# AkshayJha22/Cross-Sectional-Momentum-Strategy-Replication-Backtesting-Framework

Measured on AMD Instinct MI355X. Metric: asset-periods backtested/sec (1/2/4/8 GPU) + % HBM peak BW; decile match %, higher is better.
Workload: dtype f64

## Files before the change

### cross-sectional-momentum-strategy-replication-backtesting-framework_amd/csrc/scan.h

```cpp
#pragma once
#include "csm_common.h"

struct ScanLane {
  double pff;
  double psff;
  int head;
  int prev;
};

__device__ __forceinline__ void scan_init(ScanLane& s, double* ring, int RS, int W,
                                          const double* __restrict__ carry, int64_t N,
                                          int64_t a, bool live) {
  if (live && carry) {
    for (int k = 0; k < W; ++k) ring[k * RS] = carry[(int64_t)k * N + a];
    s.pff = carry[(int64_t)W * N + a];
    s.psff = carry[(int64_t)(W + 1) * N + a];
  } else {
    for (int k = 0; k < W; ++k) ring[k * RS] = qnan();
    s.pff = qnan();
    s.psff = qnan();
  }
  s.head = 0;
  s.prev = -1;
}

__device__ __forceinline__ double ffill(double x, double last) { return isnan_d(x) ? last : x; }

__device__ __forceinline__ double price_step(double x, double& pff) {
  const double nx = ffill(x, pff);
  const double ret = nx / pff - 1.0;
  pff = nx;
  return ret;
}

__device__ __forceinline__ void lds_push(double* ring, int RS, int W, int& head, double fct) {
  ring[head * RS] = fct;
  head = (head + 1 == W) ? 0 : head + 1;
}

template <int JC = 0>
__device__ __forceinline__ double lds_prod(const double* ring, int RS, int W, int J, int idx) {
  double acc = ring[idx * RS];
  if constexpr (JC > 0) {
    double f[JC];
#pragma unroll
    for (int k = 1; k < JC; ++k) {
      idx = (idx + 1 == W) ? 0 : idx + 1;
      f[k] = ring[idx * RS];
    }
#pragma unroll
    for (int k = 1; k < JC; ++k) acc = acc * f[k];
  } else {
    for (int k = 1; k < J; ++k) {
      idx = (idx + 1 == W) ? 0 : idx + 1;
      acc = acc * ring[idx * RS];
    }
  }
  return acc;
}

template <int RW>
__device__ __forceinline__ void reg_push(double (&f)[RW], double fct, bool on = true) {
#pragma unroll
  for (int k = 0; k + 1 < RW; ++k) f[k] = on ? f[k + 1] : f[k];
  f[RW - 1] = on ? fct : f[RW - 1];
}

template <int RW>
__device__ __forceinline__ double reg_prod(const double (&f)[RW], int J) {
  double acc = f[0];
#pragma unroll
  for (int k = 1; k < RW; ++k)
    if (k < J) acc = acc * f[k];
  return acc;
}

template <int RW, bool FIX>
__device__ __forceinline__ double mj_window(const double (&f)[RW], int q, int lo, int hi) {
  if constexpr (FIX) {
    constexpr int Jq[4] = {3, 6, 9, 12};
    double acc = 0.0;
#pragma unroll
    for (int qq = 0; qq < 4; ++qq) {
      if (qq != q) continue;
      const int l = RW - Jq[qq] - 1;
      double a = f[l];
#pragma unroll
      for (int k = l + 1; k < RW - 1; ++k) a = a * f[k];
      acc = a;
    }
    return acc;
  }
  double acc = 1.0;
#pragma unroll
  for (int k = 0; k < RW; ++k) acc = (k >= lo && k < hi) ? acc * f[k] : acc;
  return acc;
}

__device__ __forceinline__ double subset_ret(double ps_new, double psff) {
  return ps_new / psff - 1.0;
}

template <class Settle>
__device__ __forceinline__ bool rank_step(double x, double mom, int m, double& psff, int& prev,
                                          Settle settle) {
  const bool ranked = !isnan_d(mom);
  const double ps_new = ffill(x, psff);
  if (prev >= 0) settle(prev, subset_ret(ps_new, psff));
  if (ranked) {
    psff = ps_new;
    prev = m;
    return false;
  }
  prev = -1;
  return true;
}

__device__ __forceinline__ double pending_finish(double x, double psff) {
  return is_absent(x) ? qnan() : subset_ret(ffill(x, psff), psff);
}

__device__ __forceinline__ void scan_finish(ScanLane& s, double* ring, int RS, int W, int64_t N,
                                            int64_t a, double* __restrict__ NR,
                                            const double* __restrict__ next_pm,
                                            double* __restrict__ carry_out) {
  if (s.prev >= 0)
    NR[(int64_t)s.prev * N + a] = next_pm ? pending_finish(next_pm[a], s.psff) : qnan();
  if (carry_out) {
    int idx = s.head;
    for (int k = 0; k < W; ++k) {
      carry_out[(int64_t)k * N + a] = ring[idx * RS];
      idx = (idx + 1 == W) ? 0 : idx + 1;
    }
    carry_out[(int64_t)W * N + a] = s.pff;
    carry_out[(int64_t)(W + 1) * N + a] = s.psff;
  }
}

template <int JC = 0>
__device__ __forceinline__ double lds_push_mom(ScanLane& s, double* ring, int RS, int W, int J,
                                               double fct) {
  lds_push(ring, RS, W, s.head, fct);
  return lds_prod<JC>(ring, RS, W, J, s.head) - 1.0;
}

template <class Ring>
__device__ __forceinline__ double scan_step_on(ScanLane& s, double x, int m, int64_t N, int64_t a,
                                               double* __restrict__ R, double* __restrict__ M,
                                               double* __restrict__ NR, Ring push_prod) {
  const double NaN = qnan();
  const int64_t o = (int64_t)m * N + a;
  if (is_absent(x)) {
    if (R) R[o] = NaN;
    M[o] = NaN;
    NR[o] = NaN;
    return NaN;
  }
  const double ret = price_step(x, s.pff);
  const double mom = push_prod(1.0 + ret);
  if (rank_step(x, mom, m, s.psff, s.prev,
                [&](int row, double nr) { NR[(int64_t)row * N + a] = nr; }))
    NR[o] = NaN;
  if (R) R[o] = ret;
  M[o] = mom;
  return mom;
}

__device__ __forceinline__ void store_pair(double* p, double v0, double v1) {
  *reinterpret_cast<double2*>(p) = make_double2(v0, v1);
}

__device__ __forceinline__ void store_next_ret_pair(double* __restrict__ NR, int64_t N,
                                                    int64_t a0, int64_t o, const int (&wp)[2],
                                                    const double (&vp)[2], const bool (&wc)[2]) {
  const double NaN = qnan();
  if (wp[0] >= 0 && wp[0] == wp[1]) {
    store_pair(NR + (int64_t)wp[0] * N + a0, vp[0], vp[1]);
  } else {
    if (wp[0] >= 0) NR[(int64_t)wp[0] * N + a0] = vp[0];
    if (wp[1] >= 0) NR[(int64_t)wp[1] * N + a0 + 1] = vp[1];
  }
  if (wc[0] && wc[1]) {
    store_pair(NR + o, NaN, NaN);
  } else {
    if (wc[0]) NR[o] = NaN;
    if (wc[1]) NR[o + 1] = NaN;
  }
}

__device__ __forceinline__ void chunk_range(int T_m, int G, int g, int& m0, int& m1) {
  const int base = T_m / G, rem = T_m % G;
  m0 = g * base + (g < rem ? g : rem);
  m1 = m0 + base + (g < rem ? 1 : 0);
}

template <int JC = 0>
__device__ __forceinline__ double scan_step(ScanLane& s, double x, int m, double* ring, int RS,
                                            int W, int J, int64_t N, int64_t a,
                                            double* __restrict__ R, double* __restrict__ M,
                                            double* __restrict__ NR) {
  return scan_step_on(s, x, m, N, a, R, M, NR,
                      [&](double fct) { return lds_push_mom<JC>(s, ring, RS, W, J, fct); });
}

template <int JC = 0>
__device__ __forceinline__ void scan_step_pair(ScanLane (&s)[2], const double (&x)[2], int m,
                                               double* ring0, int RS, int W, int J, int64_t N,
                                               int64_t a0, double* __restrict__ R,
                                               double* __restrict__ M, double* __restrict__ NR,
                                               double (&mom)[2]) {
  const double NaN = qnan();
  double ret[2];
  int wp[2];
  double vp[2];
  bool wc[2];
#pragma unroll
  for (int c = 0; c < 2; ++c) {
    wp[c] = -1;
    vp[c] = NaN;
    if (is_absent(x[c])) {
      ret[c] = NaN; mom[c] = NaN; wc[c] = true;
      continue;
    }
    ret[c] = price_step(x[c], s[c].pff);
    mom[c] = lds_push_mom<JC>(s[c], ring0 + c, RS, W, J, 1.0 + ret[c]);
    const bool ranked = !isnan_d(mom[c]);
    const double ps_new = ffill(x[c], s[c].psff);
    if (s[c].prev >= 0) { wp[c] = s[c].prev; vp[c] = subset_ret(ps_new, s[c].psff); }
    if (ranked) {
      s[c].psff = ps_new;
      s[c].prev = m;
      wc[c] = false;
    } else {
      s[c].prev = -1;
      wc[c] = true;
    }
  }
  const int64_t o = (int64_t)m * N + a0;
  if (R) store_pair(R + o, ret[0], ret[1]);
  store_pair(M + o, mom[0], mom[1]);
  store_next_ret_pair(NR, N, a0, o, wp, vp, wc);
}

__device__ __forceinline__ void scan_shadow(ScanLane& s, double x, int m, double* ring, int RS,
                                            int W, int J) {
  if (is_absent(x)) return;
  const double ret = price_step(x, s.pff);
  const double mom = lds_push_mom(s, ring, RS, W, J, 1.0 + ret);
  rank_step(x, mom, m, s.psff, s.prev, [](int, double) {});
}

template <int VEC> struct RowT;
template <> struct RowT<1> { typedef double T; };
template <> struct RowT<2> { typedef double2 T; };
__device__ __forceinline__ double comp(double v, int) { return v; }
__device__ __forceinline__ double comp(double2 v, int k) { return k == 0 ? v.x : v.y; }

template <int WR, int JC = 0>
__device__ __forceinline__ double scan_step_reg(ScanLane& s, double x, int m, double (&fr)[WR],
                                                int J, int64_t N, int64_t a,
                                                double* __restrict__ R, double* __restrict__ M,
                                                double* __restrict__ NR) {
  return scan_step_on(s, x, m, N, a, R, M, NR, [&](double fct) {
    reg_push(fr, fct);
    return reg_prod(fr, JC > 0 ? JC : J) - 1.0;
  });
}
```

### cross-sectional-momentum-strategy-replication-backtesting-framework_amd/csrc/signal.hip

```cpp
#include "csm_common.h"
#include "scan.h"
#include "shard.h"


#define PROBE_M 8
#define PROBE_DEN 8
__device__ __forceinline__ bool tail_probe(const double* __restrict__ P,
                                           const int64_t* __restrict__ month_start, int T_m,
                                           int64_t N, int64_t T_d) {
  static_assert(PROBE_M == 8, "the month spacing is a shift");
  const int lane = threadIdx.x & 63;
  const int64_t cs = N / 128;
  double x[PROBE_M][2];
  bool in[PROBE_M];
#pragma unroll
  for (int i = 0; i < PROBE_M; ++i) {
    const int m = (int)(((int64_t)(2 * i + 1) * T_m) >> 4);
    const int64_t d0 = month_start[m] < 0 ? 0 : month_start[m];
    const int64_t d1 = month_start[m + 1] < T_d ? month_start[m + 1] : T_d;
    in[i] = d1 > d0;
#pragma unroll
    for (int j = 0; j < 2; ++j)
      x[i][j] = in[i] ? P[(d1 - 1) * N + (2 * lane + j) * cs] : 0.0;
  }
  int gaps = 0, tot = 0;
#pragma unroll
  for (int i = 0; i < PROBE_M; ++i)
#pragma unroll
    for (int j = 0; j < 2; ++j) {
      gaps += __popcll(__ballot(in[i] && !(x[i][j] == x[i][j])));
      tot += in[i] ? 64 : 0;
    }
  return gaps * PROBE_DEN <= tot;
}

struct HaloArgs {
  int H, F, before, after;
  uint8_t* flags;
};
#define HALO_BATCH 8
template <int MAXD, int VEC, int NBUF, int BW, bool SH, bool BL, int JC = 0, bool HALO = false>
__global__ __launch_bounds__(64 * BW) void k_signal(
    const double* __restrict__ P, const int64_t* __restrict__ month_start, int T_m, int64_t N,
    int J, int skip, double* __restrict__ PMo, double* __restrict__ R, double* __restrict__ M,
    double* __restrict__ NR, const double* __restrict__ carry, const double* __restrict__ next_pm,
    double* __restrict__ carry_out, int64_t T_d, uint16_t* __restrict__ IDS, HaloArgs ha,
    int probe) {
  static_assert(!HALO || (SH && VEC == 2), "the halo prologue: shard passes, paired lanes");
  if (probe && tail_probe(P, month_start, T_m, N, T_d)) return;
  typedef typename RowT<VEC>::T VT;
  extern __shared__ __attribute__((aligned(16))) double ring_lds[];
  const int W = J + skip;
  const int tid = threadIdx.x;
  const int64_t a0 = ((int64_t)blockIdx.x * 64 * BW + tid) * VEC;
  const bool live = a0 < N;
  const int RS = 64 * VEC * BW;
  ScanLane sl[VEC];
  int* shc = reinterpret_cast<int*>(ring_lds + W * RS);
#pragma unroll
  for (int k = 0; k < VEC; ++k) {
    scan_init(sl[k], ring_lds + VEC * tid + k, RS, W, HALO ? nullptr : carry, N, a0 + k, live);
    if (SH) {
      shc[VEC * tid + k] = 0;
      shc[RS + VEC * tid + k] = -1;
      shc[2 * RS + VEC * tid + k] = -1;
    }
  }
  double npmh[VEC];
  if constexpr (HALO) {
    constexpr int HU = HALO_BATCH;
    const int64_t* ms = month_start;
    const int H = ha.H, F = ha.F, HF = H + F;
    const int64_t as = live ? a0 : 0;
    const int lane = tid & 63, wv = tid >> 6;
    const int64_t aw = a0 - 2 * lane;
    double* hpw = ring_lds + (size_t)W * RS + (size_t)(3 * RS) / 2;
    uint16_t* wl = reinterpret_cast<uint16_t*>(hpw + HU * RS) + wv * (HU * 128);
    int nh[VEC], fv[VEC], lv[VEC];
#pragma unroll
    for (int c = 0; c < VEC; ++c) { nh[c] = 0; fv[c] = -1; lv[c] = -1; npmh[c] = absent_val(); }
    for (int j0 = 0; j0 < HF; j0 += HU) {
      double2 xl[HU];
#pragma unroll
      for (int u = 0; u < HU; ++u) {
        const int j = j0 + u;
        const int m = j < H ? j : j + T_m;
        xl[u] = make_double2(absent_val(), absent_val());
        if (j < HF) {
          const int64_t d0 = ms[m], d1 = ms[m + 1];
          if (d1 > d0) xl[u] = *reinterpret_cast<const double2*>(P + (d1 - 1) * N + as);
        }
      }
      int nit = 0;
#pragma unroll
      for (int u = 0; u < HU; ++u) {
        *reinterpret_cast<double2*>(hpw + u * RS + 2 * tid) = xl[u];
#pragma unroll
        for (int c = 0; c < VEC; ++c) {
          const double x = comp(xl[u], c);
          const bool need = live && j0 + u < HF && !(x == x);
          const uint64_t mk = __ballot(need);
          if (need) wl[nit + lane_prefix(mk)] = (uint16_t)(u * 128 + 2 * lane + c);
          nit += __popcll(mk);
        }
      }
      __builtin_amdgcn_wave_barrier();
      for (int it0 = 0; it0 < nit; it0 += 128) {
        int item[2], u[2];
        int64_t d0[2], d1[2];
        double xs[2][HALO_WALK];
#pragma unroll
        for (int h = 0; h < 2; ++h) {
          const int it = it0 + 64 * h + lane;
          item[h] = it < nit ? (int)wl[it] : -1;
          u[h] = item[h] >> 7;
          const int j = j0 + (item[h] < 0 ? 0 : u[h]);
          const int m = j < H ? j : j + T_m;
          d0[h] = ms[m];
          d1[h] = ms[m + 1];
          const int64_t a = aw + (item[h] & 127);
#pragma unroll
          for (int k = 0; k < HALO_WALK; ++k) {
            const int64_t d = d1[h] - 2 - k;
            xs[h][k] = (item[h] >= 0 && d >= d0[h]) ? P[d * N + a] : absent_val();
          }
        }
#pragma unroll
        for (int h = 0; h < 2; ++h) {
          if (item[h] < 0) continue;
          const int64_t a = aw + (item[h] & 127);
          const double xlast = hpw[u[h] * RS + 128 * wv + (item[h] & 127)];
          bool p = !is_absent(xlast), got = false;
          double x = 0.0;
#pragma unroll
          for (int k = 0; k < HALO_WALK; ++k) {
            if (!got && xs[h][k] == xs[h][k]) { x = xs[h][k]; got = true; }
            p |= !is_absent(xs[h][k]);
          }
          if (!got && d1[h] - 1 - HALO_WALK > d0[h]) {
            const double y = halo_month_price(P, d0[h], d1[h] - 1 - HALO_WALK, N, a);
            if (y == y) { x = y; got = true; }
            p |= !is_absent(y);
          }
          hpw[u[h] * RS + 128 * wv + (item[h] & 127)] = got ? x : (p ? qnan() : absent_val());
        }
      }
      __syncthreads();
#pragma unroll
      for (int u = 0; u < HU; ++u) {
        const int j = j0 + u;
        if (j >= HF) break;
#pragma unroll
        for (int c = 0; c < VEC; ++c) {
          const double x = hpw[u * RS + 2 * tid + c];
          if (j < H) {
            if (live && !is_absent(x)) {
              if (!isnan_d(x)) { if (fv[c] < 0) fv[c] = nh[c]; lv[c] = nh[c]; }
              ++nh[c];
              scan_shadow(sl[c], x, j, ring_lds + VEC * tid + c, RS, W, J);
            }
          } else if (is_absent(npmh[c])) {
            npmh[c] = x;
          }
        }
      }
      __syncthreads();
    }
#pragma unroll
    for (int c = 0; c < VEC; ++c) {
      sl[c].prev = -1;
      uint8_t fl = 0;
      if (ha.before && !(fv[c] >= 0 && lv[c] - fv[c] >= W)) fl |= 1;
      if (ha.after && is_absent(npmh[c])) fl |= 2;
      if (live && ha.flags) ha.flags[a0 + c] = fl;
    }
    month_start += H;
  }
  const double* base = P + (live ? a0 : 0);
  const int64_t rstride = N;
  static_assert(!BL || VEC == 2, "buffer loads: paired lanes");
  const int voff = (int)((live ? a0 : 0) * 8);
  auto load_month = [&](VT (&buf)[MAXD], int mm) {
    mm = mm < T_m ? mm : T_m - 1;
    const int64_t f0 = month_start[mm], nn = month_start[mm + 1] - f0;
    if constexpr (BL) {
      typedef unsigned int u32x4 __attribute__((ext_vector_type(4)));
      const __amdgpu_buffer_rsrc_t rs = __builtin_amdgcn_make_buffer_rsrc(
          (void*)(P + f0 * N), (short)0, (int)(nn * N * 8), 0x00020000);
#pragma unroll
      for (int k = 0; k < MAXD; ++k) {
        const u32x4 w = __builtin_amdgcn_raw_buffer_load_b128(rs, voff + k * (int)(N * 8), 0, 0);
        buf[k] = *reinterpret_cast<const VT*>(&w);
      }
    } else {
      const int64_t pad = nn > 0 ? nn - 1 : (f0 > 0 ? -1 : 0);
#pragma unroll
      for (int k = 0; k < MAXD; ++k)
        buf[k] = *reinterpret_cast<const VT*>(base + (f0 + (k < nn ? k : pad)) * rstride);
    }
  };
  auto process = [&](const VT (&X)[MAXD], int m) {
    double pm[VEC];
    const int nnm = (int)(month_start[m + 1] - month_start[m]);
#pragma unroll
    for (int c = 0; c < VEC; ++c) {
      double last = 0.0;
      bool p = false, v = false;
#pragma unroll
      for (int k = 0; k < MAXD; ++k) {
        const double x = comp(X[k], c);
        const bool in = BL ? k < nnm : nnm > 0;
        const bool ok = in && x == x;
        p |= in && !is_absent(x);
        v |= ok;
        last = ok ? x : last;
      }
      pm[c] = p ? (v ? last : qnan()) : absent_val();
      if (SH && p) {
        int* q = shc + VEC * tid + c;
        q[0] += 1;
        if (q[RS] < 0) q[RS] = m;
        q[2 * RS] = m;
      }
    }
    if (live) {
      if (PMo && (!SH || shard_pm_kept(m, T_m, W))) {
        if (VEC == 2) *reinterpret_cast<double2*>(PMo + (int64_t)m * N + a0) = make_double2(pm[0], pm[VEC - 1]);
        else PMo[(int64_t)m * N + a0] = pm[0];
      }
      double mom[VEC];
      if constexpr (VEC == 2) {
        scan_step_pair<JC>(reinterpret_cast<ScanLane (&)[2]>(sl), reinterpret_cast<const double (&)[2]>(pm),
                       m, ring_lds + VEC * tid, RS, W, J, N, a0, R, M, NR,
                       reinterpret_cast<double (&)[2]>(mom));
      } else {
#pragma unroll
        for (int c = 0; c < VEC; ++c)
          mom[c] = scan_step(sl[c], pm[c], m, ring_lds + VEC * tid + c, RS, W, J, N, a0 + c, R, M, NR);
      }
      if (IDS) {
        if (VEC == 2)
          *reinterpret_cast<uint32_t*>(IDS + (int64_t)m * N + a0) =
              csm_fid(mom[0]) | (csm_fid(mom[VEC - 1]) << 16);
        else
          IDS[(int64_t)m * N + a0] = (uint16_t)csm_fid(mom[0]);
      }
    }
  };
  static_assert(NBUF == 2 || NBUF == 4, "two or four month buffers");
  VT A[MAXD], B[MAXD];
  if (NBUF == 2) {
    load_month(A, 0);
    for (int m = 0; m < T_m; m += 2) {
      load_month(B, m + 1);
      process(A, m);
      load_month(A, m + 2);
      if (m + 1 < T_m) process(B, m + 1);
    }
  } else {
    VT C[MAXD], D[MAXD];
    load_month(A, 0);
    load_month(B, 1);
    load_month(C, 2);
    for (int m = 0; m < T_m; m += 4) {
      load_month(D, m + 3);
      process(A, m);
      load_month(A, m + 4);
      if (m + 1 < T_m) process(B, m + 1);
      load_month(B, m + 5);
      if (m + 2 < T_m) process(C, m + 2);
      load_month(C, m + 6);
      if (m + 3 < T_m) process(D, m + 3);
    }
  }
  if (live) {
#pragma unroll
    for (int k = 0; k < VEC; ++k) {
      if constexpr (HALO) {
        if (sl[k].prev >= 0)
          NR[(int64_t)sl[k].prev * N + a0 + k] = pending_finish(npmh[k], sl[k].psff);
      } else {
        scan_finish(sl[k], ring_lds + VEC * tid + k, RS, W, N, a0 + k, NR, next_pm,
                    SH ? nullptr : carry_out);
      }
      if (SH) {
        const int* q = shc + VEC * tid + k;
        carry_out[a0 + k] = (double)q[0];
        carry_out[N + a0 + k] = (double)sl[k].prev;
        carry_out[2 * N + a0 + k] = sl[k].psff;
        carry_out[3 * N + a0 + k] = (double)q[RS];
        carry_out[4 * N + a0 + k] = (double)q[2 * RS];
      }
    }
  }
}

#define TAIL_U 8
#define TAIL_BACK 3

template <int MAXD, int BW, int JC>
__global__ __launch_bounds__(64 * BW) void k_signal_tail(
    const double* __restrict__ P, const int64_t* __restrict__ month_start, int T_m, int64_t N,
    int J, int skip, double* __restrict__ PMo, double* __restrict__ R, double* __restrict__ M,
    double* __restrict__ NR, const double* __restrict__ carry, const double* __restrict__ next_pm,
    double* __restrict__ carry_out, int64_t T_d, uint16_t* __restrict__ IDS,
    int probe) {
  if (probe && !tail_probe(P, month_start, T_m, N, T_d)) return;
  extern __shared__ __attribute__((aligned(16))) double ring_lds[];
  constexpr int U = TAIL_U, RS = 64 * BW, WA = 64;
  const int W = J + skip;
  const int tid = threadIdx.x, lane = tid & 63, wv = tid >> 6;
  const int64_t a0 = (int64_t)blockIdx.x * RS + tid;
  const bool live = a0 < N;
  const int64_t as = live ? a0 : 0;
  const int64_t aw = a0 - lane;
  const int64_t* ms = month_start;
  double* hp = ring_lds + (size_t)W * RS;
  double* hpw = hp + WA * wv;
  uint16_t* wl = reinterpret_cast<uint16_t*>(hp + U * RS) + wv * (2 * U * WA);
  uint16_t* wl2 = wl + U * WA;
  ScanLane sl;
  scan_init(sl, ring_lds + tid, RS, W, carry, N, a0, live);
  if (aw >= N) return;

  auto month_rows = [&](int m, int64_t& d0, int64_t& d1) {
    d0 = ms[m];
    d1 = ms[m + 1];
    d0 = d0 < 0 ? 0 : d0;
    d1 = d1 < T_d ? d1 : T_d;
  };
  auto load_last = [&](double (&xl)[U], int m0) {
#pragma unroll
    for (int u = 0; u < U; ++u) {
      xl[u] = absent_val();
      if (m0 + u < T_m) {
        int64_t d0, d1;
        month_rows(m0 + u, d0, d1);
        if (d1 > d0) xl[u] = P[(d1 - 1) * N + as];
      }
    }
  };
  auto fold = [&](double y, double& x, bool& got, bool& p) {
    if (!got && y == y) { x = y; got = true; }
    p |= !is_absent(y);
  };
  constexpr int K = MAXD - 1;
  struct Walk {
    int item, u, col;
    int64_t d0, d1;
    bool act;
  };
  auto issue = [&](auto& xs, Walk& w, const uint16_t* list, int it, int n, int m0) {
    constexpr int KK = sizeof(xs) / sizeof(double);
    w.act = it < n;
    w.item = w.act ? (int)list[it] : 0;
    w.u = w.item / WA;
    w.col = w.item % WA;
    month_rows(m0 + w.u, w.d0, w.d1);
    const int64_t a = aw + w.col;
#pragma unroll
    for (int k = 0; k < KK; ++k) {
      const int64_t d = w.d1 - 2 - k;
      xs[k] = (w.act && d >= w.d0) ? P[d * N + a] : absent_val();
    }
  };
  auto finish_back = [&](const double (&xs)[TAIL_BACK], const Walk& w, int& nb) {
    bool p = true, got = false;
    double x = 0.0;
#pragma unroll
    for (int k = 0; k < TAIL_BACK; ++k) fold(xs[k], x, got, p);
    const bool more = w.act && !got && w.d1 - 2 - TAIL_BACK >= w.d0;
    if (w.act && !more) hpw[w.u * RS + w.col] = got ? x : qnan();
    const uint64_t mk = __ballot(more);
    if (more) wl2[nb + lane_prefix(mk)] = (uint16_t)w.item;
    nb += __popcll(mk);
  };
  auto finish_month = [&](const double (&xs)[K], const Walk& w) {
    bool p = !is_absent(hpw[w.u * RS + w.col]), got = false;
    double x = 0.0;
#pragma unroll
    for (int k = 0; k < K; ++k) fold(xs[k], x, got, p);
    if (w.act) hpw[w.u * RS + w.col] = got ? x : (p ? qnan() : absent_val());
  };
  auto walk_months = [&](int i0, int n, int m0) {
    double XS[K], XT[K];
    Walk wb, wc;
    const bool two = i0 + 64 < n;
    issue(XS, wb, wl2, i0 + lane, n, m0);
    if (two) issue(XT, wc, wl2, i0 + 64 + lane, n, m0);
    finish_month(XS, wb);
    if (two) finish_month(XT, wc);
  };

  double xa[U], xb[U];
  load_last(xa, 0);
  for (int m0 = 0; m0 < T_m; m0 += U) {
    load_last(xb, m0 + U);
    int na = 0, nb = 0;
#pragma unroll
    for (int u = 0; u < U; ++u) {
      hp[u * RS + tid] = xa[u];
      bool in = false;
      if (m0 + u < T_m) {
        int64_t d0, d1;
        month_rows(m0 + u, d0, d1);
        in = d1 > d0;
      }
      const double x = xa[u];
      const bool need = live && in && !(x == x);
      const bool nb_ = need && is_absent(x), na_ = need && !nb_;
      const uint64_t mka = __ballot(na_), mkb = __ballot(nb_);
      const int item = u * WA + lane;
      if (na_) wl[na + lane_prefix(mka)] = (uint16_t)item;
      if (nb_) wl2[nb + lane_prefix(mkb)] = (uint16_t)item;
      na += __popcll(mka);
      nb += __popcll(mkb);
    }
    __builtin_amdgcn_wave_barrier();
    if (na + nb > 0) {
      double xs[TAIL_BACK];
      Walk wa;
      int db = nb < 128 ? nb : 128;
      issue(xs, wa, wl, lane, na, m0);
      walk_months(0, db, m0);
      finish_back(xs, wa, nb);
      for (int it0 = 64; it0 < na; it0 += 64) {
        issue(xs, wa, wl, it0 + lane, na, m0);
        finish_back(xs, wa, nb);
      }
      __builtin_amdgcn_wave_barrier();
      for (; db < nb; db += 128) walk_months(db, nb, m0);
    }
    __builtin_amdgcn_wave_barrier();
#pragma unroll 1
    for (int u = 0; u < U; ++u) {
      const int m = m0 + u;
      if (m >= T_m) break;
      if (!live) continue;
      const double pm = hp[u * RS + tid];
      if (PMo) PMo[(int64_t)m * N + a0] = pm;
      const double mom = scan_step<JC>(sl, pm, m, ring_lds + tid, RS, W, J, N, a0, R, M, NR);
      if (IDS) IDS[(int64_t)m * N + a0] = (uint16_t)csm_fid(mom);
    }
    __builtin_amdgcn_wave_barrier();
#pragma unroll
    for (int u = 0; u < U; ++u) xa[u] = xb[u];
  }
  if (live) scan_finish(sl, ring_lds + tid, RS, W, N, a0, NR, next_pm, carry_out);
}

static int g_tune_signal_vec = 2;
static int g_tune_signal_bwf = 0;
static int g_tune_signal_tail = 2;
static int g_tune_signal_j12 = 1;
#define SIGNAL_BWF_MIN_N (180 * 512)
static const TuneKnob g_knobs[] = {
    {"signal_vec", &g_tune_signal_vec, [](int v) { return v == 1 || v == 2; }},
    {"signal_bwf", &g_tune_signal_bwf, [](int v) { return v == 0 || v == 1 || v == 4; }},
    {"signal_j12", &g_tune_signal_j12, [](int v) { return v == 0 || v == 1; }},
    {"signal_tail", &g_tune_signal_tail, [](int v) { return v >= 0 && v <= 2; }},
};
int csm_tune_signal(const char* key, int value) { return tune_set(g_knobs, key, value); }

int signal_launch(csm_ctx* ctx, const char* who, const double* P, int64_t T_d, int64_t N,
                  const int64_t* month_start, int32_t T_m, int32_t max_month_days, int32_t J,
                  int32_t skip, double* PM, double* R, double* M, double* NR, const double* carry,
                  const double* next_pm, double* carry_out, bool sh, uint16_t* ids,
                  const HaloArgs* halo) {
  int r = prep(ctx);
  if (r) return r;
  if (sh && (!PM || !carry_out || T_m < 1))
    return set_err(ctx, CSM_E_INVAL, "%s: a shard pass needs PM and state, and at least one month",
                   who);
  if (!P || !month_start || !M || !NR || N <= 0 || T_d < 0 || T_m < 0 || J < 1 || skip < 0 ||
      J + skip > 256 || max_month_days < 1)
    return set_err(ctx, CSM_E_INVAL, "%s: bad arguments (N=%lld T_m=%d J=%d skip=%d)", who,
                   (long long)N, T_m, J, skip);
  if (max_month_days > 32)
    return set_err(ctx, CSM_E_INVAL, "%s: months longer than 32 days are not supported "
                   "(use csm_month_end + csm_momentum)", who);
  if (T_m == 0) return CSM_OK;
  if (T_d == 0)
    return set_err(ctx, CSM_E_INVAL, "%s: %d months and no day row", who, T_m);
  const int W = J + skip;
  const bool can2 = (N % 2 == 0) && aligned16(P) && (!PM || aligned16(PM)) && aligned16(M) &&
                    aligned16(NR) && (!R || aligned16(R));
  const int vec = (g_tune_signal_vec == 1 || !can2) ? 1 : 2;
  const size_t tlds = (size_t)(W + TAIL_U) * 128 * sizeof(double) + (size_t)2 * TAIL_U * 128 * sizeof(uint16_t);
  int tail = (!sh && !halo && can2 && tlds <= 160 * 1024) ? g_tune_signal_tail : 0;
  if (tail == 2 && N < (int64_t)SIGNAL_BWF_MIN_N) tail = 1;
  int probe_ = tail == 2;
  if (tail != 0) {
    const bool d23 = max_month_days <= 23, j12 = J == 12;
    const void* fn =
        d23 ? (j12 ? (const void*)k_signal_tail<23, 2, 12> : (const void*)k_signal_tail<23, 2, 0>)
            : (j12 ? (const void*)k_signal_tail<32, 2, 12> : (const void*)k_signal_tail<32, 2, 0>);
    if (tlds > 65536)
      HIP_CHECK(ctx, hipFuncSetAttribute(fn, hipFuncAttributeMaxDynamicSharedMemorySize, (int)tlds));
    const unsigned blocks = (unsigned)((N + 127) / 128);
    int T_m_ = T_m, J_ = J, skip_ = skip;
    int64_t N_ = N, T_d_ = T_d;
    void* args[] = {(void*)&P, (void*)&month_start, &T_m_, &N_, &J_, &skip_, (void*)&PM, (void*)&R,
                    (void*)&M, (void*)&NR, (void*)&carry, (void*)&next_pm, (void*)&carry_out, &T_d_,
                    (void*)&ids, &probe_};
    HIP_CHECK(ctx, hipLaunchKernel(fn, dim3(blocks), dim3(128), args, tlds, ctx->stream));
    LAUNCH_CHECK(ctx, who);
    if (tail == 1) return CSM_OK;
  }
  const bool fits4 = vec == 2 && max_month_days <= 23 && N * 8 * 32 < ((int64_t)1 << 31);
  const bool wide4 = fits4 && (g_tune_signal_bwf == 4 ||
                               (g_tune_signal_bwf == 0 && N >= (int64_t)SIGNAL_BWF_MIN_N));
  const int bw = wide4 ? 4 : 1;
  const size_t lds = (size_t)W * 64 * vec * bw * sizeof(double) +
                     (sh ? (size_t)3 * 64 * vec * bw * sizeof(int) : 0) +
                     (halo ? (size_t)HALO_BATCH * 64 * vec * bw * sizeof(double) +
                             (size_t)bw * HALO_BATCH * 128 * sizeof(uint16_t) : 0);
  const unsigned blocks = (unsigned)((N / vec + 64 * bw - 1) / (64 * bw));
  const void* fn = nullptr;
#define SIG1(V, SH_)                                                                            \
  (max_month_days <= 23 && V == 2 ? (const void*)k_signal<23, V, 4, 1, SH_, false>              \
   : max_month_days <= 24         ? (const void*)k_signal<24, V, 4, 1, SH_, false>              \
                                  : (const void*)k_signal<32, V, 4, 1, SH_, false>)
  const bool j12 = sh && J == 12 && g_tune_signal_j12;
  if (halo && !(sh && wide4))
    return set_err(ctx, CSM_E_INVAL, "%s: the fused halo prologue runs in the wide shard kernel "
                   "(even N >= %d, months of <= 23 days); use csm_shard_halo + "
                   "csm_signal_shard_halo", who, SIGNAL_BWF_MIN_N);
  if (halo)
    fn = j12 ? (const void*)k_signal<23, 2, 2, 4, true, true, 12, true>
             : (const void*)k_signal<23, 2, 2, 4, true, true, 0, true>;
  else if (wide4 && j12)
    fn = (const void*)k_signal<23, 2, 2, 4, true, true, 12>;
  else if (wide4)
    fn = sh ? (const void*)k_signal<23, 2, 2, 4, true, true> : (const void*)k_signal<23, 2, 2, 4, false, true>;
  else if (vec == 2)
    fn = sh ? SIG1(2, true) : SIG1(2, false);
  else
    fn = sh ? SIG1(1, true) : SIG1(1, false);
#undef SIG1
  if (lds > 65536)
    HIP_CHECK(ctx, hipFuncSetAttribute(fn, hipFuncAttributeMaxDynamicSharedMemorySize, (int)lds));
  {
    int T_m_ = T_m, J_ = J, skip_ = skip;
    int64_t N_ = N, T_d_ = T_d;
    HaloArgs ha = halo ? *halo : HaloArgs{0, 0, 0, 0, nullptr};
    void* args[] = {(void*)&P, (void*)&month_start, &T_m_, &N_, &J_, &skip_, (void*)&PM, (void*)&R,
                    (void*)&M, (void*)&NR, (void*)&carry, (void*)&next_pm, (void*)&carry_out, &T_d_,
                    (void*)&ids, (void*)&ha, &probe_};
    HIP_CHECK(ctx, hipLaunchKernel(fn, dim3(blocks), dim3(64 * bw), args, lds, ctx->stream));
  }
  LAUNCH_CHECK(ctx, who);
  return CSM_OK;
}

extern "C" {

int csm_signal(csm_ctx* ctx, const double* P, int64_t T_d, int64_t N, const int64_t* month_start,
               int32_t T_m, int32_t max_month_days, int32_t J, int32_t skip, double* PM, double* R,
               double* M, double* NR, const double* carry, const double* next_pm,
               double* carry_out) {
  return signal_launch(ctx, "csm_signal", P, T_d, N, month_start, T_m, max_month_days, J,
                       skip, PM, R, M, NR, carry, next_pm, carry_out);
}

int csm_signal_ids(csm_ctx* ctx, const double* P, int64_t T_d, int64_t N,
                   const int64_t* month_start, int32_t T_m, int32_t max_month_days,
                   int32_t min_month_days, int32_t J, int32_t skip, double* PM, double* R,
                   double* M, double* NR, uint16_t* ids) {
  if (!ids || (N % 4) != 0 || ((uintptr_t)ids & 7u) != 0)
    return set_err(ctx, CSM_E_INVAL, "csm_signal_ids: ids must be non-NULL and 8-B aligned, N %% 4 == 0 "
                   "(N=%lld)", (long long)N);
  (void)min_month_days;
  return signal_launch(ctx, "csm_signal_ids", P, T_d, N, month_start, T_m, max_month_days, J,
                       skip, PM, R, M, NR, nullptr, nullptr, nullptr, false, ids);
}

int csm_signal_shard(csm_ctx* ctx, const double* P, int64_t T_d, int64_t N,
                     const int64_t* month_start, int32_t T_m, int32_t max_month_days, int32_t J,
                     int32_t skip, double* PM, double* R, double* M, double* NR, double* state) {
  return signal_launch(ctx, "csm_signal_shard", P, T_d, N, month_start, T_m,
                       max_month_days, J, skip, PM, R, M, NR, nullptr, nullptr, state, true);
}

int csm_signal_shard_ids(csm_ctx* ctx, const double* P, int64_t T_d, int64_t N,
                         const int64_t* month_start, int32_t T_m, int32_t max_month_days,
                         int32_t J, int32_t skip, double* PM, double* R, double* M, double* NR,
                         double* state, uint16_t* ids) {
  if (!ids || (N % 4) != 0 || ((uintptr_t)ids & 7u) != 0)
    return set_err(ctx, CSM_E_INVAL, "csm_signal_shard_ids: needs ids, N %% 4 == 0, 8-B aligned ids");
  return signal_launch(ctx, "csm_signal_shard_ids", P, T_d, N, month_start, T_m,
                       max_month_days, J, skip, PM, R, M, NR, nullptr, nullptr, state, true, ids);
}

int csm_signal_halo(csm_ctx* ctx, const double* P, int64_t T_d, int64_t N,
                    const int64_t* month_start, int32_t H, int32_t T_m, int32_t F, int32_t before,
                    int32_t after, int32_t max_month_days, int32_t J, int32_t skip, double* PM,
                    double* R, double* M, double* NR, double* state, uint16_t* ids,
                    uint8_t* flags) {
  if (!flags || H < 0 || F < 0 || F > 8 || J + skip > 64)
    return set_err(ctx, CSM_E_INVAL, "csm_signal_halo: bad arguments (flags [N], H >= 0, "
                   "0 <= F <= 8, J + skip <= 64)");
  if (ids && ((N % 4) != 0 || ((uintptr_t)ids & 7u) != 0))
    return set_err(ctx, CSM_E_INVAL, "csm_signal_halo: ids need N %% 4 == 0, 8-B alignment");
  const HaloArgs ha{H, F, before ? 1 : 0, after ? 1 : 0, flags};
  return signal_launch(ctx, "csm_signal_halo", P, T_d, N, month_start, T_m, max_month_days, J,
                       skip, PM, R, M, NR, nullptr, nullptr, state, true, ids, &ha);
}

int csm_signal_shard_halo(csm_ctx* ctx, const double* P, int64_t T_d, int64_t N,
                          const int64_t* month_start, int32_t T_m, int32_t max_month_days,
                          int32_t J, int32_t skip, const double* carry, const double* next_pm,
                          double* PM, double* R, double* M, double* NR, double* state,
                          uint16_t* ids) {
  if (!carry || !next_pm)
    return set_err(ctx, CSM_E_INVAL, "csm_signal_shard_halo: needs the halo's carry and next_pm");
  if (ids && ((N % 4) != 0 || ((uintptr_t)ids & 7u) != 0))
    return set_err(ctx, CSM_E_INVAL, "csm_signal_shard_halo: ids need N %% 4 == 0, 8-B alignment");
  return signal_launch(ctx, "csm_signal_shard_halo", P, T_d, N, month_start, T_m, max_month_days,
                       J, skip, PM, R, M, NR, carry, next_pm, state, true, ids);
}

}
```

Measured before the change: 822.5 billion.

## Batch the tail kernel's per-month scan across eight months with an enlarged ring

Replaces the serial per-month scan_step loop in the tail kernel with scan_step_batch, which processes U=8 months at once. It precomputes head/tail ring indices, pushes all factors, then computes the J-window products for all months in parallel. The LDS ring is enlarged to S=W+U-1 slots so that the batched pushes do not overwrite windows still being read, and the ring is moved after the month/list buffers. The last-price loads are also made branchless so the U gathers can issue together. The goal is to break the month-to-month dependency chain and expose ILP, at the cost of more LDS, more registers and more complex wraparound logic.

```diff
diff --git a/cross-sectional-momentum-strategy-replication-backtesting-framework_amd/csrc/scan.h b/cross-sectional-momentum-strategy-replication-backtesting-framework_amd/csrc/scan.h
--- a/cross-sectional-momentum-strategy-replication-backtesting-framework_amd/csrc/scan.h
+++ b/cross-sectional-momentum-strategy-replication-backtesting-framework_amd/csrc/scan.h
@@ -26,9 +26,10 @@
 
 __device__ __forceinline__ double ffill(double x, double last) { return isnan_d(x) ? last : x; }
 
+__device__ __forceinline__ double price_ret(double nx, double pff) { return nx / pff - 1.0; }
 __device__ __forceinline__ double price_step(double x, double& pff) {
   const double nx = ffill(x, pff);
-  const double ret = nx / pff - 1.0;
+  const double ret = price_ret(nx, pff);
   pff = nx;
   return ret;
 }
@@ -123,14 +124,15 @@
 __device__ __forceinline__ void scan_finish(ScanLane& s, double* ring, int RS, int W, int64_t N,
                                             int64_t a, double* __restrict__ NR,
                                             const double* __restrict__ next_pm,
-                                            double* __restrict__ carry_out) {
+                                            double* __restrict__ carry_out, int S = 0) {
+  if (S == 0) S = W;
   if (s.prev >= 0)
     NR[(int64_t)s.prev * N + a] = next_pm ? pending_finish(next_pm[a], s.psff) : qnan();
   if (carry_out) {
     int idx = s.head;
     for (int k = 0; k < W; ++k) {
       carry_out[(int64_t)k * N + a] = ring[idx * RS];
-      idx = (idx + 1 == W) ? 0 : idx + 1;
+      idx = (idx + 1 == S) ? 0 : idx + 1;
     }
     carry_out[(int64_t)W * N + a] = s.pff;
     carry_out[(int64_t)(W + 1) * N + a] = s.psff;
@@ -201,6 +203,137 @@
                                             double* __restrict__ NR) {
   return scan_step_on(s, x, m, N, a, R, M, NR,
                       [&](double fct) { return lds_push_mom<JC>(s, ring, RS, W, J, fct); });
+}
+
+template <int U>
+__device__ __forceinline__ void held(double (&v)[U]) {
+#pragma unroll
+  for (int u = 0; u < U; ++u) asm volatile("" : "+v"(v[u]));
+}
+
+template <int U, int JC = 0>
+__device__ __forceinline__ void scan_step_batch(ScanLane& s, const double (&x)[U], int m0, int nm,
+                                                bool live, double* ring, int RS, int W, int S,
+                                                int J, int64_t N, int64_t a,
+                                                double* __restrict__ R, double* __restrict__ M,
+                                                double* __restrict__ NR, double (&mom)[U]) {
+  const double NaN = qnan();
+  const int SB = S * RS;
+  bool pr[U];
+  double nx[U], den[U];
+  int tl[U], hd[U];
+  {
+    double pff = s.pff;
+    int head = s.head * RS;
+    int tail = head + W * RS;
+    tail = tail >= SB ? tail - SB : tail;
+#pragma unroll
+    for (int u = 0; u < U; ++u) {
+      pr[u] = live && u < nm && !is_absent(x[u]);
+      nx[u] = ffill(x[u], pff);
+      den[u] = pff;
+      pff = pr[u] ? nx[u] : pff;
+      tl[u] = tail;
+      const int h1 = head + RS == SB ? 0 : head + RS, t1 = tail + RS == SB ? 0 : tail + RS;
+      head = pr[u] ? h1 : head;
+      tail = pr[u] ? t1 : tail;
+      hd[u] = head;
+    }
+    s.pff = pff;
+    s.head = head / RS;
+  }
+  double ret[U];
+#pragma unroll
+  for (int u = 0; u < U; ++u) ret[u] = price_ret(nx[u], den[u]);
+  held(ret);
+#pragma unroll
+  for (int u = 0; u < U; ++u) ring[tl[u]] = 1.0 + ret[u];
+  double acc[U];
+  if constexpr (JC > 0) {
+    const double* p0[U];
+    const double* p1[U];
+    int kw[U];
+#pragma unroll
+    for (int u = 0; u < U; ++u) {
+      p0[u] = ring + hd[u];
+      p1[u] = p0[u] - SB;
+      kw[u] = SB - hd[u];
+      acc[u] = *p0[u];
+    }
+    double f[U], g[U];
+#pragma unroll
+    for (int u = 0; u < U; ++u) f[u] = (RS >= kw[u] ? p1[u] : p0[u])[RS];
+#pragma unroll
+    for (int k = 1; k < JC; ++k) {
+#pragma unroll
+      for (int u = 0; u < U; ++u)
+        g[u] = k + 1 < JC ? ((k + 1) * RS >= kw[u] ? p1[u] : p0[u])[(k + 1) * RS] : 0.0;
+#pragma unroll
+      for (int u = 0; u < U; ++u) acc[u] = acc[u] * f[u];
+      held(acc);
+#pragma unroll
+      for (int u = 0; u < U; ++u) f[u] = g[u];
+    }
+  } else {
+    int ix[U];
+#pragma unroll
+    for (int u = 0; u < U; ++u) {
+      ix[u] = hd[u];
+      acc[u] = ring[ix[u]];
+    }
+    for (int k = 1; k < J; ++k) {
+#pragma unroll
+      for (int u = 0; u < U; ++u) {
+        ix[u] = ix[u] + RS == SB ? 0 : ix[u] + RS;
+        acc[u] = acc[u] * ring[ix[u]];
+      }
+      held(acc);
+    }
+  }
+#pragma unroll
+  for (int u = 0; u < U; ++u) mom[u] = pr[u] ? acc[u] - 1.0 : NaN;
+  int srow[U];
+  double snum[U], sden[U];
+  bool unr[U];
+  {
+    double psff = s.psff;
+    int prev = s.prev;
+#pragma unroll
+    for (int u = 0; u < U; ++u) {
+      const bool ranked = pr[u] && !isnan_d(mom[u]);
+      snum[u] = ffill(x[u], psff);
+      sden[u] = psff;
+      srow[u] = pr[u] ? prev : -1;
+      unr[u] = !ranked;
+      psff = ranked ? snum[u] : psff;
+      prev = pr[u] ? (ranked ? m0 + u : -1) : prev;
+    }
+    s.psff = psff;
+    s.prev = prev;
+  }
+  double nr[U];
+  bool other = false;
+#pragma unroll
+  for (int u = 0; u < U; ++u)
+    other |= srow[u] >= 0 && !(__double_as_longlong(snum[u]) == __double_as_longlong(nx[u]) &&
+                               __double_as_longlong(sden[u]) == __double_as_longlong(den[u]));
+  if (__ballot(other) != 0) {
+#pragma unroll
+    for (int u = 0; u < U; ++u) nr[u] = subset_ret(snum[u], sden[u]);
+    held(nr);
+  } else {
+#pragma unroll
+    for (int u = 0; u < U; ++u) nr[u] = ret[u];
+  }
+#pragma unroll
+  for (int u = 0; u < U; ++u) {
+    if (!(live && u < nm)) continue;
+    const int64_t o = (int64_t)(m0 + u) * N + a;
+    if (R) R[o] = pr[u] ? ret[u] : NaN;
+    M[o] = mom[u];
+    if (srow[u] >= 0) NR[(int64_t)srow[u] * N + a] = nr[u];
+    if (unr[u]) NR[o] = NaN;
+  }
 }
 
 template <int JC = 0>
diff --git a/cross-sectional-momentum-strategy-replication-backtesting-framework_amd/csrc/signal.hip b/cross-sectional-momentum-strategy-replication-backtesting-framework_amd/csrc/signal.hip
--- a/cross-sectional-momentum-strategy-replication-backtesting-framework_amd/csrc/signal.hip
+++ b/cross-sectional-momentum-strategy-replication-backtesting-framework_amd/csrc/signal.hip
@@ -306,19 +306,22 @@
     double* __restrict__ carry_out, int64_t T_d, uint16_t* __restrict__ IDS,
     int probe) {
   if (probe && !tail_probe(P, month_start, T_m, N, T_d)) return;
-  extern __shared__ __attribute__((aligned(16))) double ring_lds[];
+  extern __shared__ __attribute__((aligned(16))) double tail_lds[];
   constexpr int U = TAIL_U, RS = 64 * BW, WA = 64;
-  const int W = J + skip;
+  const int W = J + skip, S = W + U - 1;
   const int tid = threadIdx.x, lane = tid & 63, wv = tid >> 6;
   const int64_t a0 = (int64_t)blockIdx.x * RS + tid;
   const bool live = a0 < N;
   const int64_t as = live ? a0 : 0;
   const int64_t aw = a0 - lane;
   const int64_t* ms = month_start;
-  double* hp = ring_lds + (size_t)W * RS;
+  double* hp = tail_lds;
   double* hpw = hp + WA * wv;
   uint16_t* wl = reinterpret_cast<uint16_t*>(hp + U * RS) + wv * (2 * U * WA);
   uint16_t* wl2 = wl + U * WA;
+  constexpr int LISTS = 2 * U * RS * (int)sizeof(uint16_t) / (int)sizeof(double);
+  static_assert(U * RS + LISTS >= (JC - 1) * RS, "a wrapped window's pointer leaves the array");
+  double* ring_lds = hp + U * RS + LISTS;
   ScanLane sl;
   scan_init(sl, ring_lds + tid, RS, W, carry, N, a0, live);
   if (aw >= N) return;
@@ -330,15 +333,18 @@
     d1 = d1 < T_d ? d1 : T_d;
   };
   auto load_last = [&](double (&xl)[U], int m0) {
+    int64_t d1[U];
+    bool in[U];
 #pragma unroll
     for (int u = 0; u < U; ++u) {
-      xl[u] = absent_val();
-      if (m0 + u < T_m) {
-        int64_t d0, d1;
-        month_rows(m0 + u, d0, d1);
-        if (d1 > d0) xl[u] = P[(d1 - 1) * N + as];
-      }
-    }
+      int64_t d0;
+      month_rows(m0 + u < T_m ? m0 + u : T_m - 1, d0, d1[u]);
+      in[u] = m0 + u < T_m && d1[u] > d0;
+    }
+#pragma unroll
+    for (int u = 0; u < U; ++u) xl[u] = P[(in[u] ? d1[u] - 1 : 0) * N + as];
+#pragma unroll
+    for (int u = 0; u < U; ++u) xl[u] = in[u] ? xl[u] : absent_val();
   };
   auto fold = [&](double y, double& x, bool& got, bool& p) {
     if (!got && y == y) { x = y; got = true; }
@@ -432,21 +438,26 @@
       for (; db < nb; db += 128) walk_months(db, nb, m0);
     }
     __builtin_amdgcn_wave_barrier();
-#pragma unroll 1
-    for (int u = 0; u < U; ++u) {
-      const int m = m0 + u;
-      if (m >= T_m) break;
-      if (!live) continue;
-      const double pm = hp[u * RS + tid];
-      if (PMo) PMo[(int64_t)m * N + a0] = pm;
-      const double mom = scan_step<JC>(sl, pm, m, ring_lds + tid, RS, W, J, N, a0, R, M, NR);
-      if (IDS) IDS[(int64_t)m * N + a0] = (uint16_t)csm_fid(mom);
+    {
+      const int nm = T_m - m0 < U ? T_m - m0 : U;
+      double pm[U], mom[U];
+#pragma unroll
+      for (int u = 0; u < U; ++u) pm[u] = hp[u * RS + tid];
+      scan_step_batch<U, JC>(sl, pm, m0, nm, live, ring_lds + tid, RS, W, S, J, N, a0, R, M, NR,
+                             mom);
+#pragma unroll
+      for (int u = 0; u < U; ++u) {
+        if (!(live && u < nm)) continue;
+        const int64_t o = (int64_t)(m0 + u) * N + a0;
+        if (PMo) PMo[o] = pm[u];
+        if (IDS) IDS[o] = (uint16_t)csm_fid(mom[u]);
+      }
     }
     __builtin_amdgcn_wave_barrier();
 #pragma unroll
     for (int u = 0; u < U; ++u) xa[u] = xb[u];
   }
-  if (live) scan_finish(sl, ring_lds + tid, RS, W, N, a0, NR, next_pm, carry_out);
+  if (live) scan_finish(sl, ring_lds + tid, RS, W, N, a0, NR, next_pm, carry_out, S);
 }
 
 static int g_tune_signal_vec = 2;
@@ -486,7 +497,8 @@
   const bool can2 = (N % 2 == 0) && aligned16(P) && (!PM || aligned16(PM)) && aligned16(M) &&
                     aligned16(NR) && (!R || aligned16(R));
   const int vec = (g_tune_signal_vec == 1 || !can2) ? 1 : 2;
-  const size_t tlds = (size_t)(W + TAIL_U) * 128 * sizeof(double) + (size_t)2 * TAIL_U * 128 * sizeof(uint16_t);
+  const size_t tlds = (size_t)(W + TAIL_U - 1 + TAIL_U) * 128 * sizeof(double) +
+                      (size_t)2 * TAIL_U * 128 * sizeof(uint16_t);
   int tail = (!sh && !halo && can2 && tlds <= 160 * 1024) ? g_tune_signal_tail : 0;
   if (tail == 2 && N < (int64_t)SIGNAL_BWF_MIN_N) tail = 1;
   int probe_ = tail == 2;
```

After: 853.6 billion (median of 6 runs). 1.04x the previous value.
